# 12334zq/optical-flow-1

Hardware: AMD Instinct MI355X
Metric: Mpix*warp-iters/s, TV-L1 1920x1080 5-scale (higher is better)
Workload: dtype f64; 1 GPU; tvl1flow 1920x1080 pair (synthetic P1), nscales=5 warps=5 tau=0.25 lambda=0.15 theta=0.3 zfactor=0.5 epsilon=0.01; one pair per step per GPU; workload_name=1080p, arithmetic_mode=tolerance, pairs_per_gpu=1040, pairs_in_flight_per_gpu=64, lockstep_group=16, streams_per_gpu=4, distinct_pairs=8

## Files before the change

optical-flow-1_amd/csrc/ofx_ctx.cpp:

```cpp
#include "ofx_internal.h"

#include <cstdarg>
#include <cstdlib>
#include <new>

static const size_t kSlabAlign = 256;
static const size_t kMinSlab = 32u << 20;
static const size_t kMaxSlabs = 24;

int ofx_fail(ofx_ctx *ctx, int status, const char *fmt, ...)
{
    if (ctx) {
        va_list ap;
        va_start(ap, fmt);
        vsnprintf(ctx->errmsg, sizeof(ctx->errmsg), fmt, ap);
        va_end(ap);
    }
    return status;
}

extern "C" const char *ofx_strerror(int status)
{
    switch (status) {
    case OFX_OK:        return "ok";
// ... 47 lines not shown
    ctx->rows_per_wave = 0;
    ctx->rows_per_wave2 = 0;
    ctx->fuse2 = 1;
    ctx->store_a = 1;
    ctx->concurrency = 1;
    ctx->lockstep = 0;
    ctx->warp_lds = 1;
    ctx->gauss_fused = 1;
    ctx->relaxed_dual = 0;
    ctx->tile = 0;
    ctx->tile_max_px = 0;
    ctx->nt_stores = 0;
    ctx->chunk = 0;
    ctx->spin_us = 150;
    ctx->rows_slots = 0;
    ctx->rof_pipe = 1;
    ctx->rof_window = 0;
    ctx->chi_fuse = 1;
    ctx->fuse3 = 2;
    ctx->fuse3_min_px = 0.0;
    ctx->fuse3_cursor = 1;
    ctx->fuse3_afac1 = 0;
    ctx->fuse3_afac2 = 0;
    ctx->rows_per_wave3 = 0;
    ctx->rows3_max = 32;
    ctx->fixed_work = 0;
    ctx->sor_exact = 1;
    ctx->sor_batch = 0;
    ctx->sor_fuse = 0;
    ctx->sor_tile = 0;
    ctx->sor_tile_w = 0;
    ctx->sor_wave_levels = 1;
    ctx->sor_wave_p = 0;
    ctx->sor_window = 0;
    ctx->sor_rows = 0;
    ctx->sor_spw = 0;
    ctx->sor_lds = 1;
    ctx->mem_budget = 0;
    ctx->input = OFX_IN_STORAGE;
    ctx->input_vec = 1;
    ctx->input_lut = 1;
    ctx->poll_seq = 0;
    ctx->errmsg[0] = 0;
    ctx->expo_host_ms = 0.0;
    memset(&ctx->stats, 0, sizeof(ctx->stats));

// ... 167 lines not shown
    if (!strcmp(name, "input_vec")) { ctx->input_vec = value != 0; return OFX_OK; }
    if (!strcmp(name, "input_lut")) { ctx->input_lut = value != 0; return OFX_OK; }
    if (!strcmp(name, "fuse2")) { ctx->fuse2 = value != 0; return OFX_OK; }
    if (!strcmp(name, "store_a")) {
        if (value != 0 && value != 1 && value != 2) return ofx_fail(ctx, OFX_ERR_ARG, "store_a must be 0, 1 or 2");
        ctx->store_a = (int) value;
        return OFX_OK;
    }
    if (!strcmp(name, "rows_slots")) { ctx->rows_slots = (int) value; return OFX_OK; }
    if (!strcmp(name, "rof_pipe")) { ctx->rof_pipe = value != 0; return OFX_OK; }
    if (!strcmp(name, "rof_window")) {
        if (value != 0 && value != 24 && value != 10) return ofx_fail(ctx, OFX_ERR_ARG, "rof_window must be 0, 10 or 24");
        ctx->rof_window = (int) value;
        return OFX_OK;
    }
    if (!strcmp(name, "chi_fuse")) { ctx->chi_fuse = value != 0; return OFX_OK; }
    if (!strcmp(name, "fuse3")) {
        if (value != 0 && value != 1 && value != 2) return ofx_fail(ctx, OFX_ERR_ARG, "fuse3 must be 0, 1 or 2");
        ctx->fuse3 = (int) value;
        return OFX_OK;
    }
    if (!strcmp(name, "fuse3_min_px")) { ctx->fuse3_min_px = value; return OFX_OK; }
    if (!strcmp(name, "fuse3_cursor")) { ctx->fuse3_cursor = value != 0; return OFX_OK; }
    if (!strcmp(name, "fuse3_afac1")) { ctx->fuse3_afac1 = value; return value >= 0 ? OFX_OK : ofx_fail(ctx, OFX_ERR_ARG, "fuse3_afac1 < 0"); }
    if (!strcmp(name, "fuse3_afac2")) { ctx->fuse3_afac2 = value; return value >= 0 ? OFX_OK : ofx_fail(ctx, OFX_ERR_ARG, "fuse3_afac2 < 0"); }
    if (!strcmp(name, "rows_per_wave3")) { ctx->rows_per_wave3 = (int) value; return OFX_OK; }
    if (!strcmp(name, "rows3_max")) { ctx->rows3_max = (int) value; return OFX_OK; }
    if (!strcmp(name, "spin_us")) {
        if (value < 0 || value > 1e6) return ofx_fail(ctx, OFX_ERR_ARG, "spin_us out of range");
        ctx->spin_us = (int) value;
        return OFX_OK;
    }
    if (!strcmp(name, "chunk")) {
        if (value < 0 || value > OFX_TVL1_MAX_ITERATIONS) return ofx_fail(ctx, OFX_ERR_ARG, "chunk out of range");
        ctx->chunk = (int) value;
        return OFX_OK;
    }
    return ofx_fail(ctx, OFX_ERR_ARG, "unknown option '%s'", name);
}

extern "C" int ofx_get_stats(const ofx_ctx *ctx, ofx_stats *out)
{
    if (!ctx || !out) return OFX_ERR_ARG;
    *out = ctx->stats;
    return OFX_OK;
}

void ofx_arena_reset(ofx_ctx *ctx)
// ... 47 lines not shown
```

optical-flow-1_amd/csrc/ofx_internal.h:

```cpp
#pragma once

#include <hip/hip_runtime.h>

#include <cstddef>
#include <cstdint>
#include <cstdio>
#include <cstring>
#include <chrono>
#include <vector>

#include "ofx.h"

#define OFX_NSHARD 64
#define OFX_NPOLL  4
#define OFX_MAX_GROUP 16

struct OfxIterState {
    int    n;
    int    done;
    double error;
    int    apred;
    int    seq;
    int    unit, k0, ucnt;
};
// ... 29 lines not shown
    OfxIterState *h_state;
    double       *h_aux;
    hipEvent_t    ev_poll[OFX_NPOLL];
    hipEvent_t    ev_t0, ev_t1;

    int profile;
    int rows_per_wave;
    int rows_per_wave2;
    int fuse2;
    int store_a;
    int concurrency;
    int lockstep;
    int nt_stores;
    int relaxed_dual;
    int tile;
    double tile_max_px;
    int gauss_fused;
    int warp_lds;
    int chunk;
    int fuse3;
    double fuse3_min_px;
    int fuse3_cursor;
    double fuse3_afac1, fuse3_afac2;
    int rows_per_wave3;
    int rows3_max;
    int chi_fuse;
    int rof_window;
    int rof_pipe;
    int rows_slots;
    int spin_us;
    int fixed_work;
    int sor_exact;
    int sor_fuse;
    int sor_tile;
    int sor_tile_w;
    int sor_wave_p;
    int sor_wave_levels;
    int sor_batch;
    int sor_window;
    int sor_rows;
    int sor_lds;
    int sor_spw;
    int input;
    int input_vec;
    int input_lut;
    double mem_budget;
// ... 73 lines not shown
```

optical-flow-1_amd/csrc/ofx_tvl1.hip:

```cpp
#include "ofx_ops.h"
#include "ofx_device.h"
#include "ofx_loop.h"

#include <atomic>
#include <chrono>
#include <cmath>
#include <thread>

#define TVL1_GRAD_IS_ZERO 1E-10
#define TVL1_PRESMOOTHING_SIGMA 0.8
#define STRIP_OUT 62

template <typename T> OFX_DEV double rnd_to(double x);
template <> OFX_DEV double rnd_to<double>(double x) { return x; }
template <> OFX_DEV double rnd_to<float>(double x) { return (double) (float) x; }

#ifdef OFX_NO_RFL
#define OFX_WAVE_UNIFORM(x) (x)
#else
#define OFX_WAVE_UNIFORM(x) __builtin_amdgcn_readfirstlane(x)
#endif
template <typename T> struct RowIn {
    double2 u, p1, p2, a;
    double r;
// ... 432 lines not shown
    RowIn<T> cur;
    if (!idle) {
        if (ys > 0) {
            up12 = ldw2(at(P1in, off - row2)).y;
            up22 = ldw2(at(P2in, off - row2)).y;
        }
        cur = tvl1_load_row<T>(Uin, P1in, P2in, A, R, off);
    }
    double e1;
    if (!tvl1_continues(prev1, prev2, k, nx * ny, eps2, e1)) return;
    if (idle) return;
    if (((amask >> g) & 1u) || tvl1_store_a(k, e1, eps2, afac))
        tvl1_iter2_march<T, NT, true, STRICT>(Uin, P1in, P2in, A, R, hu.out, h1.out, h2.out, hu.alt, h1.alt, h2.alt, err, k, gw, nx, ny,
                                      y0, yend, ys, yl, lef, rig, owner, off, so, up12, up22, cur, l_t, theta, taut);
    else
        tvl1_iter2_march<T, NT, false, STRICT>(Uin, P1in, P2in, A, R, hu.out, h1.out, h2.out, hu.alt, h1.alt, h2.alt, err, k, gw, nx, ny,
                                       y0, yend, ys, yl, lef, rig, owner, off, so, up12, up22, cur, l_t, theta, taut);
}

#ifndef STRIP3_OUT
#define STRIP3_OUT 56
#endif
#define STRIP3_HALO ((64 - STRIP3_OUT) / 2)
#ifndef OFX_ITER3_WAVES
#define OFX_ITER3_WAVES 3
#endif
template <typename T, bool NT, bool STRICT, int CNT>
OFX_DEV void tvl1_iter3_march(const typename Pix<T>::v2 *__restrict__ Uin, const typename Pix<T>::v2 *__restrict__ P1in,
                              const typename Pix<T>::v2 *__restrict__ P2in, const typename Pix<T>::v2 *__restrict__ A,
                              const T *__restrict__ R, typename Pix<T>::v2 *Uout, typename Pix<T>::v2 *P1out,
                              typename Pix<T>::v2 *P2out, double *__restrict__ err, int slot0, int slot_step, int gw, int nx,
                              int ny, int y0, int yend, int ys, int yl, bool lef, bool rig, bool owner, unsigned off, unsigned so,
                              double up12, double up22, RowIn<T> cur, double l_t, double theta, double taut)
{
    const unsigned E2 = 2 * sizeof(T);
    const unsigned row2 = (unsigned) nx * E2;
    const double2 z2 = make_double2(0.0, 0.0);
    const unsigned level_bytes = (unsigned) nx * (unsigned) ny * E2;
    const ofx_rsrc rU = make_rsrc(Uout, level_bytes), rP1 = make_rsrc(P1out, level_bytes), rP2 = make_rsrc(P2out, level_bytes);
    double accA = 0.0, accB = 0.0, accC = 0.0;
    double2 uA0 = z2, uA1 = z2, uA2 = z2;
    double2 a1 = z2, a2 = z2, a3 = z2, a4 = z2;
    double r1c = 0.0, r2c = 0.0, r3c = 0.0, r4c = 0.0;
    double2 p0a = z2, p0b = z2;
    double2 pA1a = z2, pA1b = z2, pA2a = z2, pA2b = z2;
    double2 uB0 = z2, uB1 = z2, uB2 = z2;
    double2 pB1a = z2, pB1b = z2, pB2a = z2, pB2b = z2;
    double2 uC0 = z2, uC1 = z2;
    const int nyl = ny - 1;
    const int yB0 = y0 > 0 ? y0 - 1 : 0;
    const int ylc = (yend + CNT - 1 < yl) ? yend + CNT - 1 : yl;
    const int hiA = (yend + CNT - 2 < nyl) ? yend + CNT - 2 : nyl;
    const int hiB = (yend + CNT - 3 < nyl) ? yend + CNT - 3 : nyl;
    const int hiC = (yend < nyl) ? yend : nyl;
    const int ylast = yend - 1 + (2 * CNT - 1);
#ifdef OFX_CEIL_ALU
    const unsigned off0 = off;
#endif

    auto step = [&](const int y) {
        RowIn<T> nxt = cur;
#ifdef OFX_CEIL_ALU
        if (y + 1 <= ylc) nxt = tvl1_load_row<T>(Uin, P1in, P2in, A, R, off0 + ((y & 1) ? row2 : 0u));
#else
        if (y + 1 <= ylc) nxt = tvl1_load_row<T>(Uin, P1in, P2in, A, R, off + row2);
#endif
        unsigned stu = OFX_OOB, stp = OFX_OOB;
        double2 su = z2, sp1 = z2, sp2 = z2;

        if (y <= ylc) {
            const double l11 = wave_shift_up(cur.p1.x);
            const double l21 = wave_shift_up(cur.p2.x);
            uA0 = tvl1_primal<T, STRICT>(cur.u, cur.a, cur.r, cur.p1, cur.p2, l11, l21, up12, up22, lef, rig, y == 0, y == nyl, l_t,
                                         theta);
            const bool mine = owner && y >= y0 && y < yend;
            const double dA = (uA0.x - cur.u.x) * (uA0.x - cur.u.x) + (uA0.y - cur.u.y) * (uA0.y - cur.u.y);
            accA += mine ? dA : 0.0;
            if (CNT == 1 && mine) { stu = so; su = uA0; }
        }
        double2 pAna = z2, pAnb = z2;
        if (y - 1 >= ys && y - 1 <= hiA) {
            const double n1 = wave_shift_down(uA1.x);
            const double n2 = wave_shift_down(uA1.y);
            tvl1_dual<T, STRICT>(p0a, p0b, uA1, n1, n2, uA0, rig, y - 1 == nyl, taut, pAna, pAnb);
            pAna.x = rnd_to<T>(pAna.x); pAna.y = rnd_to<T>(pAna.y);
            pAnb.x = rnd_to<T>(pAnb.x); pAnb.y = rnd_to<T>(pAnb.y);
            if (CNT == 1 && owner && y - 1 >= y0 && y - 1 < yend) { stp = so - row2; sp1 = pAna; sp2 = pAnb; }
        }
        double2 pBna = z2, pBnb = z2;
        if (CNT >= 2) {
            if (y - 2 >= yB0 && y - 2 <= hiA) {
                const double l11 = wave_shift_up(pA1a.x);
                const double l21 = wave_shift_up(pA1b.x);
                uB0 = tvl1_primal<T, STRICT>(uA2, a2, r2c, pA1a, pA1b, l11, l21, pA2a.y, pA2b.y, lef, rig, y - 2 == 0, y - 2 == nyl,
                                             l_t, theta);
                const bool mine = owner && y - 2 >= y0 && y - 2 < yend;
                const double dB = (uB0.x - uA2.x) * (uB0.x - uA2.x) + (uB0.y - uA2.y) * (uB0.y - uA2.y);
                accB += mine ? dB : 0.0;
                if (CNT == 2 && mine) { stu = so - 2 * row2; su = uB0; }
            }
            if (y - 3 >= yB0 && y - 3 <= hiB) {
                const double n1 = wave_shift_down(uB1.x);
                const double n2 = wave_shift_down(uB1.y);
                tvl1_dual<T, STRICT>(pA2a, pA2b, uB1, n1, n2, uB0, rig, y - 3 == nyl, taut, pBna, pBnb);
                pBna.x = rnd_to<T>(pBna.x); pBna.y = rnd_to<T>(pBna.y);
                pBnb.x = rnd_to<T>(pBnb.x); pBnb.y = rnd_to<T>(pBnb.y);
                if (CNT == 2 && owner && y - 3 >= y0 && y - 3 < yend) { stp = so - 3 * row2; sp1 = pBna; sp2 = pBnb; }
            }
        }
        if (CNT == 3) {
            if (y - 4 >= y0 && y - 4 <= hiC) {
                const double l11 = wave_shift_up(pB1a.x);
                const double l21 = wave_shift_up(pB1b.x);
                uC0 = tvl1_primal<T, STRICT>(uB2, a4, r4c, pB1a, pB1b, l11, l21, pB2a.y, pB2b.y, lef, rig, y - 4 == 0, y - 4 == nyl,
                                             l_t, theta);
                const bool mine = owner && y - 4 < yend;
                const double dC = (uC0.x - uB2.x) * (uC0.x - uB2.x) + (uC0.y - uB2.y) * (uC0.y - uB2.y);
                accC += mine ? dC : 0.0;
                stu = mine ? so - 4 * row2 : stu;
                su = uC0;
            }
            if (y - 5 >= y0 && y - 5 < yend) {
                const double n1 = wave_shift_down(uC1.x);
                const double n2 = wave_shift_down(uC1.y);
                tvl1_dual<T, STRICT>(pB2a, pB2b, uC1, n1, n2, uC0, rig, y - 5 == nyl, taut, sp1, sp2);
                if (owner) stp = so - 5 * row2;
            }
        }
#ifdef OFX_CEIL_ALU
        stu = OFX_OOB; stp = OFX_OOB;
#endif
        bst2<NT>(rU, stu, su, Uout);
        bst2<NT>(rP1, stp, sp1, P1out);
        bst2<NT>(rP2, stp, sp2, P2out);
        uA2 = uA1; uA1 = uA0;
        a4 = a3; a3 = a2; a2 = a1; a1 = cur.a;
        r4c = r3c; r3c = r2c; r2c = r1c; r1c = cur.r;
        p0a = cur.p1; p0b = cur.p2;
        up12 = cur.p1.y; up22 = cur.p2.y;
        pA2a = pA1a; pA2b = pA1b; pA1a = pAna; pA1b = pAnb;
        uB2 = uB1; uB1 = uB0;
        pB2a = pB1a; pB2b = pB1b; pB1a = pBna; pB1b = pBnb;
        uC1 = uC0;
        cur = nxt;
        off += row2;
        so += row2;
    };
    for (int y = ys; y <= ylast; y++) step(y);
    loop_accumulate(err, slot0, accA, gw);
    if (CNT >= 2) loop_accumulate(err, slot0 + slot_step, accB, gw);
    if (CNT == 3) loop_accumulate(err, slot0 + 2 * slot_step, accC, gw);
}

template <typename T, bool NT, bool STRICT>
__global__ __launch_bounds__(256) __attribute__((amdgpu_waves_per_eu(OFX_ITER3_WAVES, OFX_ITER3_WAVES))) void k_tvl1_iter3(
    Tri<typename Pix<T>::v2> Ut, Tri<typename Pix<T>::v2> P1t, Tri<typename Pix<T>::v2> P2t,
    const typename Pix<T>::v2 *__restrict__ Ag, const T *__restrict__ Rg, double *__restrict__ errg, int k0, int check, int slot0,
    int nx, int ny, int rows, int strips_x, int strips_pad, double l_t, double theta, double taut, double eps2, unsigned incode,
    unsigned runmask, unsigned long long nit, int err_stride, OfxLoopDev *dev, int launch, double afac1, double afac2, int max_iter)
{
    using v2 = typename Pix<T>::v2;
    const int lane = threadIdx.x & 63;
    const int gw = OFX_WAVE_UNIFORM((int) (blockIdx.x * 4 + (threadIdx.x >> 6)));
    const int g = blockIdx.y;
    if (!((runmask >> g) & 1u)) return;
    int niter = (int) ((nit >> (4 * g)) & 15ull);
    const bool scribe = dev && blockIdx.x == 0 && threadIdx.x == 0;
    if (dev) {
        k0 = dev->cursor[launch & 1][g];
        slot0 = k0;
        check = 1;
        if (scribe) {
            dev->ulog[g][launch] = k0;
            dev->cursor[(launch + 1) & 1][g] = k0;
        }
        if (k0 >= max_iter) return;
    }
    const size_t npix = (size_t) nx * ny;
    const TriSel<v2> hu = pick3(Ut, incode, g, npix), h1 = pick3(P1t, incode, g, npix), h2 = pick3(P2t, incode, g, npix);
    const v2 *__restrict__ Uin = hu.in, *__restrict__ P1in = h1.in, *__restrict__ P2in = h2.in;
    const v2 *__restrict__ A = Ag + (size_t) g * npix;
    const T *__restrict__ R = Rg + (size_t) g * npix;
    double *__restrict__ err = errg + (size_t) g * err_stride;
    double prev[3];
#pragma unroll
    for (int i = 0; i < 3; i++) prev[i] = (check && k0 - i > 0) ? loop_fetch_prev(err, k0 - i) : 0.0;

    const int band = gw / strips_pad, strip = gw % strips_pad;
    const int y0 = band * rows;
    const bool idle = (strip >= strips_x) || (y0 >= ny);
    const int yend = (y0 + rows < ny) ? y0 + rows : ny;
    const int ys = y0 > 2 ? y0 - 2 : 0;
    const int yl = (yend + 2 < ny - 1) ? yend + 2 : ny - 1;
    const int c = strip * STRIP3_OUT - STRIP3_HALO + lane;
    const int cc = c < 0 ? 0 : (c > nx - 1 ? nx - 1 : c);
    const bool lef = (c == 0), rig = (c == nx - 1);
    const bool owner = (lane >= STRIP3_HALO) && (lane < STRIP3_OUT + STRIP3_HALO) && (c < nx);
    const unsigned E2 = 2 * sizeof(T);
    const unsigned row2 = (unsigned) nx * E2;
    const unsigned off = ((unsigned) ys * nx + cc) * E2;
    const unsigned so = ((unsigned) ys * nx + (c < 0 ? 0 : c)) * E2;
    double up12 = 0.0, up22 = 0.0;
    RowIn<T> cur;
    if (!idle) {
        if (ys > 0) {
            up12 = ldw2(at(P1in, off - row2)).y;
            up22 = ldw2(at(P2in, off - row2)).y;
        }
        cur = tvl1_load_row<T>(Uin, P1in, P2in, A, R, off);
    }
    if (check) {
        double e1 = 0.0;
#pragma unroll
        for (int i = 0; i < 3; i++) {
            if (k0 - i > 0) {
                const double e = loop_error_from_sum(wave_allreduce_sum(prev[i]), nx * ny, OFX_CRIT_MEAN);
                if (!(e > eps2)) return;
                if (i == 0) e1 = e;
            }
        }
        if (dev) {
            niter = (k0 > 0 && e1 <= eps2 * afac1) ? 1 : ((k0 > 0 && e1 <= eps2 * afac2) ? 2 : 3);
            if (niter > max_iter - k0) niter = max_iter - k0;
            if (scribe) dev->cursor[(launch + 1) & 1][g] = k0 + niter;
        }
    }
    if (idle) return;
    const int step = check ? 1 : 0;
    if (niter >= 3)
        tvl1_iter3_march<T, NT, STRICT, 3>(Uin, P1in, P2in, A, R, hu.out, h1.out, h2.out, err, slot0, step, gw, nx, ny, y0, yend, ys, yl,
                                           lef, rig, owner, off, so, up12, up22, cur, l_t, theta, taut);
    else if (niter == 2)
        tvl1_iter3_march<T, NT, STRICT, 2>(Uin, P1in, P2in, A, R, hu.out, h1.out, h2.out, err, slot0, step, gw, nx, ny, y0, yend, ys, yl,
                                           lef, rig, owner, off, so, up12, up22, cur, l_t, theta, taut);
    else
        tvl1_iter3_march<T, NT, STRICT, 1>(Uin, P1in, P2in, A, R, hu.out, h1.out, h2.out, err, slot0, step, gw, nx, ny, y0, yend, ys, yl,
                                           lef, rig, owner, off, so, up12, up22, cur, l_t, theta, taut);
}

#define TILE_RH 16
template <typename T, bool STRICT, int K>
__global__ __launch_bounds__(64 * TILE_RH) void k_tvl1_tile(
    Tri<typename Pix<T>::v2> Ut, Tri<typename Pix<T>::v2> P1t, Tri<typename Pix<T>::v2> P2t,
    const typename Pix<T>::v2 *__restrict__ Ag, const T *__restrict__ Rg, double *__restrict__ errg, int k0, int check, int slot0,
    int nx, int ny, int tiles_x, double l_t, double theta, double taut, double eps2, unsigned incode, unsigned runmask,
    unsigned long long nit, int err_stride)
{
    using v2 = typename Pix<T>::v2;
    static_assert(K < 16, "4 bits of `nit` per pair");
    __shared__ double2 s_p[2][TILE_RH][64];
    __shared__ double2 s_u[2][TILE_RH][64];
    const int lane = threadIdx.x & 63, w = threadIdx.x >> 6;
    const int g = blockIdx.y;
    if (!((runmask >> g) & 1u)) return;
    const int niter = (int) ((nit >> (4 * g)) & 15ull);
    const size_t npix = (size_t) nx * ny;
    const TriSel<v2> hu = pick3(Ut, incode, g, npix), h1 = pick3(P1t, incode, g, npix), h2 = pick3(P2t, incode, g, npix);
    double *__restrict__ err = errg + (size_t) g * err_stride;
    double prev[K];
#pragma unroll
// ... 305 lines not shown

static int tvl1_pick_chunk(const ofx_ctx *ctx, int nx, int ny, int G)
{
    if (ctx->chunk > 0) return ctx->chunk;
    const double est_us = fmax(5.0, (double) nx * ny * G * 120.0 / 4.0e6);
    int c = (int) (40.0 / est_us);
    return c < 4 ? 4 : (c > 50 ? 50 : c);
}

static int tvl1_pick_tile(const ofx_ctx *ctx, int nx, int ny, int G)
{
    if (!ctx->tile || !ctx->fuse2) return 0;
    const double lim = ctx->tile_max_px > 0 ? ctx->tile_max_px : 200000.0;
    if ((double) nx * ny * G > lim) return 0;
    return ctx->tile == 6 ? 6 : 4;
}

template <typename T> struct Tvl1Level;
struct Tvl1Params;
template <typename T>
static int tvl1_run_iterations_tile(ofx_ctx *ctx, Tvl1Level<T> &L, const Tvl1Params &P, LoopSpec S, int K, int *n_out,
                                    double *err_out, float *ms_out, int *alt_out);
template <typename T>
static int tvl1_run_iterations_tri(ofx_ctx *ctx, Tvl1Level<T> &L, const Tvl1Params &P, LoopSpec S, int *n_out, double *err_out,
                                   float *ms_out, int *alt_out);

static int tvl1_pick_rows3(const ofx_ctx *ctx, int nx, int ny, int G)
{
    if (ctx->rows_per_wave3 > 0) return ctx->rows_per_wave3;
    {
        static const char *tab = getenv("OFX_ROWS3");
        for (const char *q = tab; q && *q;) {
            int lny = 0, r = 0;
            if (sscanf(q, "%d:%d", &lny, &r) == 2 && lny == ny && r > 0) return r;
            q = strchr(q, '/');
            if (q) q++;
        }
    }
    const long strips_pad = (long) ofx_cdiv(ofx_cdiv(nx, STRIP3_OUT), 4) * 4 * G;
    const int rmax = 32;
    int best = rmax;
    long best_cost = -1;
    if (ctx->concurrency > 1) {
        static const int cand[] = {2, 3, 4, 5, 6, 8, 10, 12, 14, 16, 20, 24, 28, 32, 36, 40, 48, 54, 64, 72, 80, 96};
        for (int r : cand) {
            if (r > ctx->rows3_max) break;
            const long waves = strips_pad * ofx_cdiv(ny, r);
            const long slots = ctx->rows_slots > 0 ? ctx->rows_slots : 1024;
            const long cost = ((waves + slots - 1) / slots) * (r + 7);
            if (best_cost < 0 || cost < best_cost) { best_cost = cost; best = r; }
        }
        return best;
    }
    const long slots = 1024L * OFX_ITER3_WAVES;
    for (int k = 1; k <= 4; k++) {
        for (int r = 1; r <= rmax; r++) {
            if (strips_pad * ofx_cdiv(ny, r) > k * slots) continue;
            const long cost = (long) k * (r + 7);
            if (best_cost < 0 || cost < best_cost) { best_cost = cost; best = r; }
            break;
        }
    }
    if (best < 4 && strips_pad * ofx_cdiv(ny, 4) >= 512) best = 4;
    return best;
}

template <typename T>
static int tvl1_run_iterations(ofx_ctx *ctx, Tvl1Level<T> &L, const Tvl1Params &P, int *n_out, double *err_out,
                               float *ms_out, int *alt_out = nullptr,
                               int *unit_out = nullptr)
{
    const int nx = L.nx, ny = L.ny, G = L.G;
    if ((long long) nx * ny >= (1LL << 27)) return ofx_fail(ctx, OFX_ERR_ARG, "tvl1: image larger than 2^27 pixels");
    const double l_t = P.lambda * P.theta, taut = P.tau / P.theta, theta = P.theta;
    const bool pairs = ctx->fuse2 != 0;
    const int rows = tvl1_pick_rows(ctx, nx, ny, G);
    const int strips_x = ofx_cdiv(nx, STRIP_OUT), strips_pad = ofx_cdiv(strips_x, 4) * 4;
    const unsigned gx1 = (unsigned) (strips_pad / 4) * ofx_cdiv(ny, rows);
    const dim3 block(256);
    const int rows2 = tvl1_pick_rows2(ctx, nx, ny, G);
    const int strips2_x = ofx_cdiv(nx, STRIP2_OUT), strips2_pad = ofx_cdiv(strips2_x, 4) * 4;
    const dim3 grid2((unsigned) (strips2_pad / 4) * ofx_cdiv(ny, rows2), G);
    LoopSpec S;
    S.max_iter = P.max_iter;
    S.size = nx * ny;
    S.thr = P.epsilon * P.epsilon;
    S.crit = OFX_CRIT_MEAN;
    S.chunk = tvl1_pick_chunk(ctx, nx, ny, G);
    S.fixed = P.fixed;
    S.pairs = pairs;
    const int tileK = tvl1_pick_tile(ctx, nx, ny, G);
    if (unit_out) *unit_out = tileK ? tileK : (pairs ? 2 : 1);
    if (tileK) return tvl1_run_iterations_tile<T>(ctx, L, P, S, tileK, n_out, err_out, ms_out, alt_out);
    {
        const bool strict_mode = sizeof(T) == sizeof(double) && !ctx->relaxed_dual;
        const double px = (double) nx * ny * G;
        const bool tri = ctx->fuse3 == 1 ? px >= ctx->fuse3_min_px
                                         : (ctx->fuse3 == 2 && !strict_mode && (G >= 2 || ctx->concurrency > 1) &&
                                            px >= (ctx->fuse3_min_px > 0 ? ctx->fuse3_min_px : 5e5));
        if (pairs && tri) {
            if (unit_out) *unit_out = 3;
            return tvl1_run_iterations_tri<T>(ctx, L, P, S, n_out, err_out, ms_out, alt_out);
        }
    }
    const int err_stride = (S.max_iter + 1) * OFX_NSHARD;
    const unsigned all = (G >= 32) ? 0xFFFFFFFFu : ((1u << G) - 1u);
    const bool nt_stores = ctx->nt_stores ? ctx->nt_stores == 1 : (double) nx * ny * G * 15.0 * sizeof(T) > 300e6;
    unsigned b0[OFX_MAX_GROUP];
    for (int g = 0; g < G; g++) b0[g] = L.curidx(g);
    auto code_of = [&](unsigned unit) -> unsigned {
        unsigned c = 0;
        for (int g = 0; g < G; g++) c |= ((b0[g] + unit) % 3u) << (2 * g);
        return c;
    };
    const bool sa = pairs && !P.fixed && ctx->store_a != 0;
    S.afac = sa ? (ctx->store_a == 2 ? 1e300 : 1.5) : 0.0;
    unsigned amask0 = 0;
    if (sa)
        for (int g = 0; g < G; g++)
            if (ctx->store_a == 2 || (L.last_n[g] >= 1 && L.last_n[g] <= 2)) amask0 |= 1u << g;
    const bool strict = sizeof(T) == sizeof(double) && !ctx->relaxed_dual;
    auto single = [&](unsigned incode, unsigned runmask, int check, int slot, double thr) -> int {
        auto kern = k_tvl1_iter<T, false>;
        if constexpr (sizeof(T) == sizeof(double)) { if (strict) kern = k_tvl1_iter<T, true>; }
        hipLaunchKernelGGL(kern, dim3(gx1, G), block, 0, ctx->stream, L.Ut(), L.P1t(), L.P2t(), L.A, (const T *) L.R,
// ... 82 lines not shown
        for (int g = 0; g < G; g++) {
            if (k_of[g] < 0) continue;
            const int n = k_of[g] + 1, j = (n - 1) / K;
            runmask |= 1u << g;
            incode |= ((b0[g] + (unsigned) j) % 3u) << (2 * g);
            nit |= (unsigned long long) (n - j * K) << (4 * g);
        }
        return go(0, 0, S.max_iter, -1.0, incode, runmask, nit);
    };
    int took_alt[OFX_MAX_GROUP];
    OFX_TRY(ofx_run_loop_group(ctx, S, G, launch, redo, n_out, err_out, ms_out, 0u, took_alt));
    unsigned cur = 0;
    for (int g = 0; g < G; g++) {
        const unsigned units = (unsigned) ((n_out[g] + K - 1) / K);
        cur |= ((b0[g] + units) % 3u) << (2 * g);
        L.last_n[g] = n_out[g];
        if (alt_out) alt_out[g] = 0;
    }
    L.cur = cur;
    return OFX_OK;
}

template <typename T>
static int tvl1_run_iterations_tri(ofx_ctx *ctx, Tvl1Level<T> &L, const Tvl1Params &P, LoopSpec S, int *n_out, double *err_out,
                                   float *ms_out, int *alt_out)
{
    const int nx = L.nx, ny = L.ny, G = L.G;
    const double l_t = P.lambda * P.theta, taut = P.tau / P.theta, theta = P.theta;
    const bool strict = sizeof(T) == sizeof(double) && !ctx->relaxed_dual;
    const int rows = tvl1_pick_rows3(ctx, nx, ny, G);
    const int strips_x = ofx_cdiv(nx, STRIP3_OUT), strips_pad = ofx_cdiv(strips_x, 4) * 4;
    const dim3 grid((unsigned) (strips_pad / 4) * ofx_cdiv(ny, rows), G), block(256);
    const bool nt_stores = ctx->nt_stores ? ctx->nt_stores == 1 : (double) nx * ny * G * 15.0 * sizeof(T) > 300e6;
    S.pairs = false;
    S.fuse = 3;
    S.afac = 0.0;
    const int err_stride = (S.max_iter + 1) * OFX_NSHARD;
    const unsigned all = (G >= 32) ? 0xFFFFFFFFu : ((1u << G) - 1u);
    unsigned b0[OFX_MAX_GROUP];
    for (int g = 0; g < G; g++) b0[g] = L.curidx(g);
    const bool cursor = ctx->fuse3_cursor != 0 && !S.fixed;
    const double afac2 = ctx->fuse3_afac2 > 0 ? ctx->fuse3_afac2 : 1.5, afac1 = ctx->fuse3_afac1 > 0 ? ctx->fuse3_afac1 : 1.2;
    auto go = [&](int k0, int check, int slot0, double thr, unsigned incode, unsigned runmask, unsigned long long nit, OfxLoopDev *dev,
                  int launch) -> int {
        auto kern = nt_stores ? k_tvl1_iter3<T, true, false> : k_tvl1_iter3<T, false, false>;
        if constexpr (sizeof(T) == sizeof(double)) {
            if (strict) kern = nt_stores ? k_tvl1_iter3<T, true, true> : k_tvl1_iter3<T, false, true>;
        }
        hipLaunchKernelGGL(kern, grid, block, 0, ctx->stream, L.Ut(), L.P1t(), L.P2t(), L.A, (const T *) L.R, ctx->d_err, k0, check,
                           slot0, nx, ny, rows, strips_x, strips_pad, l_t, theta, taut, thr, incode, runmask, nit, err_stride, dev, launch,
                           afac1, afac2, S.max_iter);
        OFX_LAUNCH_CHECK(ctx);
        return OFX_OK;
    };
    auto code_of_unit = [&](unsigned unit) -> unsigned {
        unsigned c = 0;
        for (int g = 0; g < G; g++) c |= ((b0[g] + unit) % 3u) << (2 * g);
        return c;
    };
    int unit_of[OFX_MAX_GROUP];
    int inside[OFX_MAX_GROUP];
    if (cursor) {
        auto launch = [&](int Lidx, double thr) -> int {
            return go(0, 1, 0, thr, code_of_unit((unsigned) Lidx), all, 0ull, reinterpret_cast<OfxLoopDev *>(ctx->d_state), Lidx);
        };
        auto redo = [&](const int *n_of, const int *k0_of, const int *u_of) -> int {
            unsigned incode = 0, runmask = 0;
            unsigned long long nit = 0;
            for (int g = 0; g < G; g++) {
                if (n_of[g] < 0) continue;
                runmask |= 1u << g;
                incode |= ((b0[g] + (unsigned) u_of[g]) % 3u) << (2 * g);
                nit |= (unsigned long long) (n_of[g] - k0_of[g]) << (4 * g);
            }
            return go(0, 0, S.max_iter, -1.0, incode, runmask, nit, nullptr, 0);
        };
        const int upc = (S.chunk + 2) / 3 < 1 ? 1 : (S.chunk + 2) / 3;
        OFX_TRY(ofx_run_loop_cursor(ctx, S, G, upc, 3, launch, redo, n_out, err_out, unit_of, inside, ms_out));
    } else {
        auto launch = [&](int k, int cnt, double thr) -> int {
            unsigned long long nit = 0;
            for (int g = 0; g < G; g++) nit |= (unsigned long long) cnt << (4 * g);
            return go(k, 1, k, thr, code_of_unit((unsigned) (k / 3)), all, nit, nullptr, 0);
        };
        auto redo = [&](const int *k_of) -> int {
            unsigned incode = 0, runmask = 0;
            unsigned long long nit = 0;
            for (int g = 0; g < G; g++) {
                if (k_of[g] < 0) continue;
                const int n = k_of[g] + 1, j = (n - 1) / 3;
                runmask |= 1u << g;
                incode |= ((b0[g] + (unsigned) j) % 3u) << (2 * g);
                nit |= (unsigned long long) (n - j * 3) << (4 * g);
            }
            return go(0, 0, S.max_iter, -1.0, incode, runmask, nit, nullptr, 0);
        };
        int took_alt[OFX_MAX_GROUP];
        OFX_TRY(ofx_run_loop_group(ctx, S, G, launch, redo, n_out, err_out, ms_out, 0u, took_alt));
        for (int g = 0; g < G; g++) {
            unit_of[g] = n_out[g] > 0 ? (n_out[g] - 1) / 3 : -1;
            inside[g] = (n_out[g] % 3 != 0 && n_out[g] != S.max_iter) ? 1 : 0;
        }
    }
    unsigned cur = 0;
    for (int g = 0; g < G; g++) {
        const unsigned units = (unsigned) (unit_of[g] + 1);
        cur |= ((b0[g] + units) % 3u) << (2 * g);
        L.last_n[g] = n_out[g];
        if (alt_out) alt_out[g] = inside[g] ? 1 : 0;
    }
    L.cur = cur;
    return OFX_OK;
}

template <typename T>
static int tvl1_single_scale_dev(ofx_ctx *ctx, Tvl1Level<T> &L, const Tvl1Params &P, int scale, ofx_stats *stats)
{
    const int nx = L.nx, ny = L.ny, G = L.G;
    const size_t n = L.n();
    const dim3 g2(ofx_cdiv(nx, OFX_WARP_BX), ofx_cdiv(ny, OFX_WARP_BY), G), b2(OFX_WARP_BX, OFX_WARP_BY);
    if (nx < 2 || ny < 2) return ofx_fail(ctx, OFX_ERR_ARG, "tvl1: level %dx%d too small", nx, ny);

    OFX_TRY(op_grad_pack<T>(ctx, L.I1, L.pa, L.pb, nx, ny, G));
    for (int h = 0; h < 3; h++) {
// ... 476 lines not shown
```

Measured before the change: 76480 Mpix*warp-iters/s.

## Add four-iteration fused TV-L1 march kernel with LDS ring for data terms

Extends the temporally fused row-marching TV-L1 iteration from three to four primal/dual iterations per launch. A new k_tvl1_iter4 kernel keeps the A and R data terms of recent rows in a shared-memory ring instead of a register shift chain, which lets it add a fourth pipeline stage with its own halo rows and error accumulator. It is selected by default for levels of at least about two million pixels when the three-iteration path would be used. The intent is to cut global memory round trips and launches per iteration, at the cost of deeper row halos (more redundant computation), extra register pressure and LDS traffic, and a coarser convergence-check granularity.

Result: faster. 78440 Mpix*warp-iters/s, median of 6 (+2.6%).

```diff
diff --git a/optical-flow-1_amd/csrc/ofx_ctx.cpp b/optical-flow-1_amd/csrc/ofx_ctx.cpp
--- a/optical-flow-1_amd/csrc/ofx_ctx.cpp
+++ b/optical-flow-1_amd/csrc/ofx_ctx.cpp
@@ -93,6 +93,9 @@
     ctx->fuse3_cursor = 1;
     ctx->fuse3_afac1 = 0;
     ctx->fuse3_afac2 = 0;
+    ctx->fuse4 = 2;
+    ctx->fuse4_min_px = 0.0;
+    ctx->fuse4_afac3 = 0;
     ctx->rows_per_wave3 = 0;
     ctx->rows3_max = 32;
     ctx->fixed_work = 0;
@@ -306,8 +309,21 @@
     }
     if (!strcmp(name, "fuse3_min_px")) { ctx->fuse3_min_px = value; return OFX_OK; }
     if (!strcmp(name, "fuse3_cursor")) { ctx->fuse3_cursor = value != 0; return OFX_OK; }
-    if (!strcmp(name, "fuse3_afac1")) { ctx->fuse3_afac1 = value; return value >= 0 ? OFX_OK : ofx_fail(ctx, OFX_ERR_ARG, "fuse3_afac1 < 0"); }
-    if (!strcmp(name, "fuse3_afac2")) { ctx->fuse3_afac2 = value; return value >= 0 ? OFX_OK : ofx_fail(ctx, OFX_ERR_ARG, "fuse3_afac2 < 0"); }
+    if (!strcmp(name, "fuse3_afac1") || !strcmp(name, "fuse3_afac2") || !strcmp(name, "fuse4_afac3")) {
+        if (!(value >= 0)) return ofx_fail(ctx, OFX_ERR_ARG, "%s < 0", name);
+        (name[10] == '1' ? ctx->fuse3_afac1 : (name[10] == '2' ? ctx->fuse3_afac2 : ctx->fuse4_afac3)) = value;
+        return OFX_OK;
+    }
+    if (!strcmp(name, "fuse4")) {
+        if (value != 0 && value != 1 && value != 2) return ofx_fail(ctx, OFX_ERR_ARG, "fuse4 must be 0, 1 or 2");
+        ctx->fuse4 = (int) value;
+        return OFX_OK;
+    }
+    if (!strcmp(name, "fuse4_min_px")) {
+        if (!(value >= 0)) return ofx_fail(ctx, OFX_ERR_ARG, "fuse4_min_px < 0");
+        ctx->fuse4_min_px = value;
+        return OFX_OK;
+    }
     if (!strcmp(name, "rows_per_wave3")) { ctx->rows_per_wave3 = (int) value; return OFX_OK; }
     if (!strcmp(name, "rows3_max")) { ctx->rows3_max = (int) value; return OFX_OK; }
     if (!strcmp(name, "spin_us")) {
diff --git a/optical-flow-1_amd/csrc/ofx_internal.h b/optical-flow-1_amd/csrc/ofx_internal.h
--- a/optical-flow-1_amd/csrc/ofx_internal.h
+++ b/optical-flow-1_amd/csrc/ofx_internal.h
@@ -75,6 +75,9 @@
     double fuse3_min_px;
     int fuse3_cursor;
     double fuse3_afac1, fuse3_afac2;
+    int fuse4;
+    double fuse4_min_px;
+    double fuse4_afac3;
     int rows_per_wave3;
     int rows3_max;
     int chi_fuse;
diff --git a/optical-flow-1_amd/csrc/ofx_tvl1.hip b/optical-flow-1_amd/csrc/ofx_tvl1.hip
--- a/optical-flow-1_amd/csrc/ofx_tvl1.hip
+++ b/optical-flow-1_amd/csrc/ofx_tvl1.hip
@@ -478,23 +478,31 @@
 #define STRIP3_OUT 56
 #endif
 #define STRIP3_HALO ((64 - STRIP3_OUT) / 2)
+#define TVL1_RING_ROWS 8
+struct Tvl1Ring {
+    double2 a[TVL1_RING_ROWS][64];
+    double  r[TVL1_RING_ROWS][64];
+};
 #ifndef OFX_ITER3_WAVES
 #define OFX_ITER3_WAVES 3
 #endif
-template <typename T, bool NT, bool STRICT, int CNT>
+template <typename T, bool NT, bool STRICT, int CNT, int N>
 OFX_DEV void tvl1_iter3_march(const typename Pix<T>::v2 *__restrict__ Uin, const typename Pix<T>::v2 *__restrict__ P1in,
                               const typename Pix<T>::v2 *__restrict__ P2in, const typename Pix<T>::v2 *__restrict__ A,
                               const T *__restrict__ R, typename Pix<T>::v2 *Uout, typename Pix<T>::v2 *P1out,
                               typename Pix<T>::v2 *P2out, double *__restrict__ err, int slot0, int slot_step, int gw, int nx,
                               int ny, int y0, int yend, int ys, int yl, bool lef, bool rig, bool owner, unsigned off, unsigned so,
-                              double up12, double up22, RowIn<T> cur, double l_t, double theta, double taut)
-{
+                              double up12, double up22, RowIn<T> cur, double l_t, double theta, double taut,
+                              Tvl1Ring *ring = nullptr)
+{
+    static_assert(CNT >= 1 && CNT <= N && (N == 3 || N == 4), "units of up to three or four iterations");
+    constexpr bool RING = CNT == 4;
     const unsigned E2 = 2 * sizeof(T);
     const unsigned row2 = (unsigned) nx * E2;
     const double2 z2 = make_double2(0.0, 0.0);
     const unsigned level_bytes = (unsigned) nx * (unsigned) ny * E2;
     const ofx_rsrc rU = make_rsrc(Uout, level_bytes), rP1 = make_rsrc(P1out, level_bytes), rP2 = make_rsrc(P2out, level_bytes);
-    double accA = 0.0, accB = 0.0, accC = 0.0;
+    double accA = 0.0, accB = 0.0, accC = 0.0, accD = 0.0;
     double2 uA0 = z2, uA1 = z2, uA2 = z2;
     double2 a1 = z2, a2 = z2, a3 = z2, a4 = z2;
     double r1c = 0.0, r2c = 0.0, r3c = 0.0, r4c = 0.0;
@@ -502,14 +510,18 @@
     double2 pA1a = z2, pA1b = z2, pA2a = z2, pA2b = z2;
     double2 uB0 = z2, uB1 = z2, uB2 = z2;
     double2 pB1a = z2, pB1b = z2, pB2a = z2, pB2b = z2;
-    double2 uC0 = z2, uC1 = z2;
+    double2 uC0 = z2, uC1 = z2, uC2 = z2;
+    double2 pC1a = z2, pC1b = z2, pC2a = z2, pC2b = z2;
+    double2 uD0 = z2, uD1 = z2;
     const int nyl = ny - 1;
-    const int yB0 = y0 > 0 ? y0 - 1 : 0;
+    const int yB0 = y0 > N - 2 ? y0 - (N - 2) : 0;
+    const int yC0 = y0 > N - 3 ? y0 - (N - 3) : 0;
     const int ylc = (yend + CNT - 1 < yl) ? yend + CNT - 1 : yl;
     const int hiA = (yend + CNT - 2 < nyl) ? yend + CNT - 2 : nyl;
     const int hiB = (yend + CNT - 3 < nyl) ? yend + CNT - 3 : nyl;
-    const int hiC = (yend < nyl) ? yend : nyl;
+    const int hiC = (yend + CNT - 4 < nyl) ? yend + CNT - 4 : nyl;
     const int ylast = yend - 1 + (2 * CNT - 1);
+    unsigned ri = 0;
 #ifdef OFX_CEIL_ALU
     const unsigned off0 = off;
 #endif
@@ -543,12 +555,20 @@
             pAnb.x = rnd_to<T>(pAnb.x); pAnb.y = rnd_to<T>(pAnb.y);
             if (CNT == 1 && owner && y - 1 >= y0 && y - 1 < yend) { stp = so - row2; sp1 = pAna; sp2 = pAnb; }
         }
+        [[maybe_unused]] const int lane = threadIdx.x & 63;
+        if constexpr (RING) {
+            ring->a[ri][lane] = cur.a;
+            ring->r[ri][lane] = cur.r;
+        }
         double2 pBna = z2, pBnb = z2;
         if (CNT >= 2) {
             if (y - 2 >= yB0 && y - 2 <= hiA) {
+                double2 ad = a2;
+                double rd = r2c;
+                if constexpr (RING) { ad = ring->a[(ri - 2u) % TVL1_RING_ROWS][lane]; rd = ring->r[(ri - 2u) % TVL1_RING_ROWS][lane]; }
                 const double l11 = wave_shift_up(pA1a.x);
                 const double l21 = wave_shift_up(pA1b.x);
-                uB0 = tvl1_primal<T, STRICT>(uA2, a2, r2c, pA1a, pA1b, l11, l21, pA2a.y, pA2b.y, lef, rig, y - 2 == 0, y - 2 == nyl,
+                uB0 = tvl1_primal<T, STRICT>(uA2, ad, rd, pA1a, pA1b, l11, l21, pA2a.y, pA2b.y, lef, rig, y - 2 == 0, y - 2 == nyl,
                                              l_t, theta);
                 const bool mine = owner && y - 2 >= y0 && y - 2 < yend;
                 const double dB = (uB0.x - uA2.x) * (uB0.x - uA2.x) + (uB0.y - uA2.y) * (uB0.y - uA2.y);
@@ -564,23 +584,56 @@
                 if (CNT == 2 && owner && y - 3 >= y0 && y - 3 < yend) { stp = so - 3 * row2; sp1 = pBna; sp2 = pBnb; }
             }
         }
-        if (CNT == 3) {
-            if (y - 4 >= y0 && y - 4 <= hiC) {
+        double2 pCna = z2, pCnb = z2;
+        if (CNT >= 3) {
+            if (y - 4 >= yC0 && y - 4 <= hiB) {
+                double2 ad = a4;
+                double rd = r4c;
+                if constexpr (RING) { ad = ring->a[(ri - 4u) % TVL1_RING_ROWS][lane]; rd = ring->r[(ri - 4u) % TVL1_RING_ROWS][lane]; }
                 const double l11 = wave_shift_up(pB1a.x);
                 const double l21 = wave_shift_up(pB1b.x);
-                uC0 = tvl1_primal<T, STRICT>(uB2, a4, r4c, pB1a, pB1b, l11, l21, pB2a.y, pB2b.y, lef, rig, y - 4 == 0, y - 4 == nyl,
+                uC0 = tvl1_primal<T, STRICT>(uB2, ad, rd, pB1a, pB1b, l11, l21, pB2a.y, pB2b.y, lef, rig, y - 4 == 0, y - 4 == nyl,
                                              l_t, theta);
-                const bool mine = owner && y - 4 < yend;
+                const bool mine = owner && y - 4 >= y0 && y - 4 < yend;
                 const double dC = (uC0.x - uB2.x) * (uC0.x - uB2.x) + (uC0.y - uB2.y) * (uC0.y - uB2.y);
                 accC += mine ? dC : 0.0;
-                stu = mine ? so - 4 * row2 : stu;
-                su = uC0;
+                if (CNT == 3) {
+                    stu = mine ? so - 4 * row2 : stu;
+                    su = uC0;
+                }
             }
-            if (y - 5 >= y0 && y - 5 < yend) {
+            if (y - 5 >= yC0 && y - 5 <= hiC) {
                 const double n1 = wave_shift_down(uC1.x);
                 const double n2 = wave_shift_down(uC1.y);
-                tvl1_dual<T, STRICT>(pB2a, pB2b, uC1, n1, n2, uC0, rig, y - 5 == nyl, taut, sp1, sp2);
-                if (owner) stp = so - 5 * row2;
+                tvl1_dual<T, STRICT>(pB2a, pB2b, uC1, n1, n2, uC0, rig, y - 5 == nyl, taut, pCna, pCnb);
+                if (CNT == 3) {
+                    sp1 = pCna; sp2 = pCnb;
+                    if (owner && y - 5 >= y0) stp = so - 5 * row2;
+                } else {
+                    pCna.x = rnd_to<T>(pCna.x); pCna.y = rnd_to<T>(pCna.y);
+                    pCnb.x = rnd_to<T>(pCnb.x); pCnb.y = rnd_to<T>(pCnb.y);
+                }
+            }
+        }
+        if constexpr (CNT == 4) {
+            if (y - 6 >= y0 && y - 6 <= hiC) {
+                const double2 ad = ring->a[(ri - 6u) % TVL1_RING_ROWS][lane];
+                const double rd = ring->r[(ri - 6u) % TVL1_RING_ROWS][lane];
+                const double l11 = wave_shift_up(pC1a.x);
+                const double l21 = wave_shift_up(pC1b.x);
+                uD0 = tvl1_primal<T, STRICT>(uC2, ad, rd, pC1a, pC1b, l11, l21, pC2a.y, pC2b.y, lef, rig, y - 6 == 0, y - 6 == nyl,
+                                             l_t, theta);
+                const bool mine = owner && y - 6 < yend;
+                const double dD = (uD0.x - uC2.x) * (uD0.x - uC2.x) + (uD0.y - uC2.y) * (uD0.y - uC2.y);
+                accD += mine ? dD : 0.0;
+                stu = mine ? so - 6 * row2 : stu;
+                su = uD0;
+            }
+            if (y - 7 >= y0 && y - 7 < yend) {
+                const double n1 = wave_shift_down(uD1.x);
+                const double n2 = wave_shift_down(uD1.y);
+                tvl1_dual<T, STRICT>(pC2a, pC2b, uD1, n1, n2, uD0, rig, y - 7 == nyl, taut, sp1, sp2);
+                if (owner) stp = so - 7 * row2;
             }
         }
 #ifdef OFX_CEIL_ALU
@@ -590,14 +643,20 @@
         bst2<NT>(rP1, stp, sp1, P1out);
         bst2<NT>(rP2, stp, sp2, P2out);
         uA2 = uA1; uA1 = uA0;
-        a4 = a3; a3 = a2; a2 = a1; a1 = cur.a;
-        r4c = r3c; r3c = r2c; r2c = r1c; r1c = cur.r;
+        if constexpr (RING) {
+            ri = (ri + 1u) % TVL1_RING_ROWS;
+        } else {
+            a4 = a3; a3 = a2; a2 = a1; a1 = cur.a;
+            r4c = r3c; r3c = r2c; r2c = r1c; r1c = cur.r;
+        }
         p0a = cur.p1; p0b = cur.p2;
         up12 = cur.p1.y; up22 = cur.p2.y;
         pA2a = pA1a; pA2b = pA1b; pA1a = pAna; pA1b = pAnb;
         uB2 = uB1; uB1 = uB0;
         pB2a = pB1a; pB2b = pB1b; pB1a = pBna; pB1b = pBnb;
-        uC1 = uC0;
+        uC2 = uC1; uC1 = uC0;
+        pC2a = pC1a; pC2b = pC1b; pC1a = pCna; pC1b = pCnb;
+        uD1 = uD0;
         cur = nxt;
         off += row2;
         so += row2;
@@ -605,15 +664,16 @@
     for (int y = ys; y <= ylast; y++) step(y);
     loop_accumulate(err, slot0, accA, gw);
     if (CNT >= 2) loop_accumulate(err, slot0 + slot_step, accB, gw);
-    if (CNT == 3) loop_accumulate(err, slot0 + 2 * slot_step, accC, gw);
-}
-
-template <typename T, bool NT, bool STRICT>
-__global__ __launch_bounds__(256) __attribute__((amdgpu_waves_per_eu(OFX_ITER3_WAVES, OFX_ITER3_WAVES))) void k_tvl1_iter3(
-    Tri<typename Pix<T>::v2> Ut, Tri<typename Pix<T>::v2> P1t, Tri<typename Pix<T>::v2> P2t,
-    const typename Pix<T>::v2 *__restrict__ Ag, const T *__restrict__ Rg, double *__restrict__ errg, int k0, int check, int slot0,
-    int nx, int ny, int rows, int strips_x, int strips_pad, double l_t, double theta, double taut, double eps2, unsigned incode,
-    unsigned runmask, unsigned long long nit, int err_stride, OfxLoopDev *dev, int launch, double afac1, double afac2, int max_iter)
+    if (CNT >= 3) loop_accumulate(err, slot0 + 2 * slot_step, accC, gw);
+    if (CNT == 4) loop_accumulate(err, slot0 + 3 * slot_step, accD, gw);
+}
+
+template <typename T, bool NT, bool STRICT, int N>
+OFX_DEV void tvl1_unit(Tri<typename Pix<T>::v2> Ut, Tri<typename Pix<T>::v2> P1t, Tri<typename Pix<T>::v2> P2t,
+                       const typename Pix<T>::v2 *__restrict__ Ag, const T *__restrict__ Rg, double *__restrict__ errg, int k0,
+                       int check, int slot0, int nx, int ny, int rows, int strips_x, int strips_pad, double l_t, double theta,
+                       double taut, double eps2, unsigned incode, unsigned runmask, unsigned long long nit, int err_stride,
+                       OfxLoopDev *dev, int launch, double afac1, double afac2, double afac3, int max_iter, Tvl1Ring *ring)
 {
     using v2 = typename Pix<T>::v2;
     const int lane = threadIdx.x & 63;
@@ -638,16 +698,16 @@
     const v2 *__restrict__ A = Ag + (size_t) g * npix;
     const T *__restrict__ R = Rg + (size_t) g * npix;
     double *__restrict__ err = errg + (size_t) g * err_stride;
-    double prev[3];
+    double prev[N];
 #pragma unroll
-    for (int i = 0; i < 3; i++) prev[i] = (check && k0 - i > 0) ? loop_fetch_prev(err, k0 - i) : 0.0;
+    for (int i = 0; i < N; i++) prev[i] = (check && k0 - i > 0) ? loop_fetch_prev(err, k0 - i) : 0.0;
 
     const int band = gw / strips_pad, strip = gw % strips_pad;
     const int y0 = band * rows;
     const bool idle = (strip >= strips_x) || (y0 >= ny);
     const int yend = (y0 + rows < ny) ? y0 + rows : ny;
-    const int ys = y0 > 2 ? y0 - 2 : 0;
-    const int yl = (yend + 2 < ny - 1) ? yend + 2 : ny - 1;
+    const int ys = y0 > N - 1 ? y0 - (N - 1) : 0;
+    const int yl = (yend + N - 1 < ny - 1) ? yend + N - 1 : ny - 1;
     const int c = strip * STRIP3_OUT - STRIP3_HALO + lane;
     const int cc = c < 0 ? 0 : (c > nx - 1 ? nx - 1 : c);
     const bool lef = (c == 0), rig = (c == nx - 1);
@@ -668,7 +728,7 @@
     if (check) {
         double e1 = 0.0;
 #pragma unroll
-        for (int i = 0; i < 3; i++) {
+        for (int i = 0; i < N; i++) {
             if (k0 - i > 0) {
                 const double e = loop_error_from_sum(wave_allreduce_sum(prev[i]), nx * ny, OFX_CRIT_MEAN);
                 if (!(e > eps2)) return;
@@ -677,21 +737,51 @@
         }
         if (dev) {
             niter = (k0 > 0 && e1 <= eps2 * afac1) ? 1 : ((k0 > 0 && e1 <= eps2 * afac2) ? 2 : 3);
+            if (N == 4 && niter == 3 && !(k0 > 0 && e1 <= eps2 * afac3)) niter = 4;
             if (niter > max_iter - k0) niter = max_iter - k0;
             if (scribe) dev->cursor[(launch + 1) & 1][g] = k0 + niter;
         }
     }
     if (idle) return;
     const int step = check ? 1 : 0;
-    if (niter >= 3)
-        tvl1_iter3_march<T, NT, STRICT, 3>(Uin, P1in, P2in, A, R, hu.out, h1.out, h2.out, err, slot0, step, gw, nx, ny, y0, yend, ys, yl,
-                                           lef, rig, owner, off, so, up12, up22, cur, l_t, theta, taut);
+    if (N == 4 && niter >= 4) {
+        if constexpr (N == 4)
+            tvl1_iter3_march<T, NT, STRICT, 4, N>(Uin, P1in, P2in, A, R, hu.out, h1.out, h2.out, err, slot0, step, gw, nx, ny, y0, yend,
+                                                  ys, yl, lef, rig, owner, off, so, up12, up22, cur, l_t, theta, taut, ring);
+    } else if (niter >= 3)
+        tvl1_iter3_march<T, NT, STRICT, 3, N>(Uin, P1in, P2in, A, R, hu.out, h1.out, h2.out, err, slot0, step, gw, nx, ny, y0, yend, ys,
+                                              yl, lef, rig, owner, off, so, up12, up22, cur, l_t, theta, taut);
     else if (niter == 2)
-        tvl1_iter3_march<T, NT, STRICT, 2>(Uin, P1in, P2in, A, R, hu.out, h1.out, h2.out, err, slot0, step, gw, nx, ny, y0, yend, ys, yl,
-                                           lef, rig, owner, off, so, up12, up22, cur, l_t, theta, taut);
+        tvl1_iter3_march<T, NT, STRICT, 2, N>(Uin, P1in, P2in, A, R, hu.out, h1.out, h2.out, err, slot0, step, gw, nx, ny, y0, yend, ys,
+                                              yl, lef, rig, owner, off, so, up12, up22, cur, l_t, theta, taut);
     else
-        tvl1_iter3_march<T, NT, STRICT, 1>(Uin, P1in, P2in, A, R, hu.out, h1.out, h2.out, err, slot0, step, gw, nx, ny, y0, yend, ys, yl,
-                                           lef, rig, owner, off, so, up12, up22, cur, l_t, theta, taut);
+        tvl1_iter3_march<T, NT, STRICT, 1, N>(Uin, P1in, P2in, A, R, hu.out, h1.out, h2.out, err, slot0, step, gw, nx, ny, y0, yend, ys,
+                                              yl, lef, rig, owner, off, so, up12, up22, cur, l_t, theta, taut);
+}
+
+template <typename T, bool NT, bool STRICT>
+__global__ __launch_bounds__(256) __attribute__((amdgpu_waves_per_eu(OFX_ITER3_WAVES, OFX_ITER3_WAVES))) void k_tvl1_iter3(
+    Tri<typename Pix<T>::v2> Ut, Tri<typename Pix<T>::v2> P1t, Tri<typename Pix<T>::v2> P2t,
+    const typename Pix<T>::v2 *__restrict__ Ag, const T *__restrict__ Rg, double *__restrict__ errg, int k0, int check, int slot0,
+    int nx, int ny, int rows, int strips_x, int strips_pad, double l_t, double theta, double taut, double eps2, unsigned incode,
+    unsigned runmask, unsigned long long nit, int err_stride, OfxLoopDev *dev, int launch, double afac1, double afac2, double afac3,
+    int max_iter)
+{
+    tvl1_unit<T, NT, STRICT, 3>(Ut, P1t, P2t, Ag, Rg, errg, k0, check, slot0, nx, ny, rows, strips_x, strips_pad, l_t, theta, taut, eps2,
+                                incode, runmask, nit, err_stride, dev, launch, afac1, afac2, afac3, max_iter, nullptr);
+}
+
+template <typename T, bool NT, bool STRICT>
+__global__ __launch_bounds__(256) __attribute__((amdgpu_waves_per_eu(OFX_ITER3_WAVES, OFX_ITER3_WAVES))) void k_tvl1_iter4(
+    Tri<typename Pix<T>::v2> Ut, Tri<typename Pix<T>::v2> P1t, Tri<typename Pix<T>::v2> P2t,
+    const typename Pix<T>::v2 *__restrict__ Ag, const T *__restrict__ Rg, double *__restrict__ errg, int k0, int check, int slot0,
+    int nx, int ny, int rows, int strips_x, int strips_pad, double l_t, double theta, double taut, double eps2, unsigned incode,
+    unsigned runmask, unsigned long long nit, int err_stride, OfxLoopDev *dev, int launch, double afac1, double afac2, double afac3,
+    int max_iter)
+{
+    __shared__ Tvl1Ring rings[4];
+    tvl1_unit<T, NT, STRICT, 4>(Ut, P1t, P2t, Ag, Rg, errg, k0, check, slot0, nx, ny, rows, strips_x, strips_pad, l_t, theta, taut, eps2,
+                                incode, runmask, nit, err_stride, dev, launch, afac1, afac2, afac3, max_iter, &rings[threadIdx.x >> 6]);
 }
 
 #define TILE_RH 16
@@ -1043,11 +1133,12 @@
 static int tvl1_run_iterations_tile(ofx_ctx *ctx, Tvl1Level<T> &L, const Tvl1Params &P, LoopSpec S, int K, int *n_out,
                                     double *err_out, float *ms_out, int *alt_out);
 template <typename T>
-static int tvl1_run_iterations_tri(ofx_ctx *ctx, Tvl1Level<T> &L, const Tvl1Params &P, LoopSpec S, int *n_out, double *err_out,
+static int tvl1_run_iterations_tri(ofx_ctx *ctx, Tvl1Level<T> &L, const Tvl1Params &P, LoopSpec S, int N, int *n_out, double *err_out,
                                    float *ms_out, int *alt_out);
 
-static int tvl1_pick_rows3(const ofx_ctx *ctx, int nx, int ny, int G)
-{
+static int tvl1_pick_rows3(const ofx_ctx *ctx, int nx, int ny, int G, int N = 3)
+{
+    const int depth = 2 * N + 1;
     if (ctx->rows_per_wave3 > 0) return ctx->rows_per_wave3;
     {
         static const char *tab = getenv("OFX_ROWS3");
@@ -1068,7 +1159,7 @@
             if (r > ctx->rows3_max) break;
             const long waves = strips_pad * ofx_cdiv(ny, r);
             const long slots = ctx->rows_slots > 0 ? ctx->rows_slots : 1024;
-            const long cost = ((waves + slots - 1) / slots) * (r + 7);
+            const long cost = ((waves + slots - 1) / slots) * (r + depth);
             if (best_cost < 0 || cost < best_cost) { best_cost = cost; best = r; }
         }
         return best;
@@ -1077,7 +1168,7 @@
     for (int k = 1; k <= 4; k++) {
         for (int r = 1; r <= rmax; r++) {
             if (strips_pad * ofx_cdiv(ny, r) > k * slots) continue;
-            const long cost = (long) k * (r + 7);
+            const long cost = (long) k * (r + depth);
             if (best_cost < 0 || cost < best_cost) { best_cost = cost; best = r; }
             break;
         }
@@ -1086,6 +1177,9 @@
     return best;
 }
 
+#ifndef TVL1_FUSE4_AUTO_PX
+#define TVL1_FUSE4_AUTO_PX 2e6
+#endif
 template <typename T>
 static int tvl1_run_iterations(ofx_ctx *ctx, Tvl1Level<T> &L, const Tvl1Params &P, int *n_out, double *err_out,
                                float *ms_out, int *alt_out = nullptr,
@@ -1119,9 +1213,12 @@
         const bool tri = ctx->fuse3 == 1 ? px >= ctx->fuse3_min_px
                                          : (ctx->fuse3 == 2 && !strict_mode && (G >= 2 || ctx->concurrency > 1) &&
                                             px >= (ctx->fuse3_min_px > 0 ? ctx->fuse3_min_px : 5e5));
-        if (pairs && tri) {
-            if (unit_out) *unit_out = 3;
-            return tvl1_run_iterations_tri<T>(ctx, L, P, S, n_out, err_out, ms_out, alt_out);
+        const bool quad = ctx->fuse4 == 1 ? px >= ctx->fuse4_min_px
+                                          : (ctx->fuse4 == 2 && tri && ctx->fuse3 == 2 &&
+                                             px >= (ctx->fuse4_min_px > 0 ? ctx->fuse4_min_px : TVL1_FUSE4_AUTO_PX));
+        if (pairs && (tri || quad)) {
+            if (unit_out) *unit_out = quad ? 4 : 3;
+            return tvl1_run_iterations_tri<T>(ctx, L, P, S, quad ? 4 : 3, n_out, err_out, ms_out, alt_out);
         }
     }
     const int err_stride = (S.max_iter + 1) * OFX_NSHARD;
@@ -1250,18 +1347,18 @@
 }
 
 template <typename T>
-static int tvl1_run_iterations_tri(ofx_ctx *ctx, Tvl1Level<T> &L, const Tvl1Params &P, LoopSpec S, int *n_out, double *err_out,
+static int tvl1_run_iterations_tri(ofx_ctx *ctx, Tvl1Level<T> &L, const Tvl1Params &P, LoopSpec S, int N, int *n_out, double *err_out,
                                    float *ms_out, int *alt_out)
 {
     const int nx = L.nx, ny = L.ny, G = L.G;
     const double l_t = P.lambda * P.theta, taut = P.tau / P.theta, theta = P.theta;
     const bool strict = sizeof(T) == sizeof(double) && !ctx->relaxed_dual;
-    const int rows = tvl1_pick_rows3(ctx, nx, ny, G);
+    const int rows = tvl1_pick_rows3(ctx, nx, ny, G, N);
     const int strips_x = ofx_cdiv(nx, STRIP3_OUT), strips_pad = ofx_cdiv(strips_x, 4) * 4;
     const dim3 grid((unsigned) (strips_pad / 4) * ofx_cdiv(ny, rows), G), block(256);
     const bool nt_stores = ctx->nt_stores ? ctx->nt_stores == 1 : (double) nx * ny * G * 15.0 * sizeof(T) > 300e6;
     S.pairs = false;
-    S.fuse = 3;
+    S.fuse = N;
     S.afac = 0.0;
     const int err_stride = (S.max_iter + 1) * OFX_NSHARD;
     const unsigned all = (G >= 32) ? 0xFFFFFFFFu : ((1u << G) - 1u);
@@ -1269,15 +1366,18 @@
     for (int g = 0; g < G; g++) b0[g] = L.curidx(g);
     const bool cursor = ctx->fuse3_cursor != 0 && !S.fixed;
     const double afac2 = ctx->fuse3_afac2 > 0 ? ctx->fuse3_afac2 : 1.5, afac1 = ctx->fuse3_afac1 > 0 ? ctx->fuse3_afac1 : 1.2;
+    const double afac3 = ctx->fuse4_afac3 > 0 ? ctx->fuse4_afac3 : afac2;
     auto go = [&](int k0, int check, int slot0, double thr, unsigned incode, unsigned runmask, unsigned long long nit, OfxLoopDev *dev,
                   int launch) -> int {
         auto kern = nt_stores ? k_tvl1_iter3<T, true, false> : k_tvl1_iter3<T, false, false>;
+        if (N == 4) kern = nt_stores ? k_tvl1_iter4<T, true, false> : k_tvl1_iter4<T, false, false>;
         if constexpr (sizeof(T) == sizeof(double)) {
             if (strict) kern = nt_stores ? k_tvl1_iter3<T, true, true> : k_tvl1_iter3<T, false, true>;
+            if (strict && N == 4) kern = nt_stores ? k_tvl1_iter4<T, true, true> : k_tvl1_iter4<T, false, true>;
         }
         hipLaunchKernelGGL(kern, grid, block, 0, ctx->stream, L.Ut(), L.P1t(), L.P2t(), L.A, (const T *) L.R, ctx->d_err, k0, check,
                            slot0, nx, ny, rows, strips_x, strips_pad, l_t, theta, taut, thr, incode, runmask, nit, err_stride, dev, launch,
-                           afac1, afac2, S.max_iter);
+                           afac1, afac2, afac3, S.max_iter);
         OFX_LAUNCH_CHECK(ctx);
         return OFX_OK;
     };
@@ -1303,31 +1403,31 @@
             }
             return go(0, 0, S.max_iter, -1.0, incode, runmask, nit, nullptr, 0);
         };
-        const int upc = (S.chunk + 2) / 3 < 1 ? 1 : (S.chunk + 2) / 3;
-        OFX_TRY(ofx_run_loop_cursor(ctx, S, G, upc, 3, launch, redo, n_out, err_out, unit_of, inside, ms_out));
+        const int upc = (S.chunk + N - 1) / N < 1 ? 1 : (S.chunk + N - 1) / N;
+        OFX_TRY(ofx_run_loop_cursor(ctx, S, G, upc, N, launch, redo, n_out, err_out, unit_of, inside, ms_out));
     } else {
         auto launch = [&](int k, int cnt, double thr) -> int {
             unsigned long long nit = 0;
             for (int g = 0; g < G; g++) nit |= (unsigned long long) cnt << (4 * g);
-            return go(k, 1, k, thr, code_of_unit((unsigned) (k / 3)), all, nit, nullptr, 0);
+            return go(k, 1, k, thr, code_of_unit((unsigned) (k / N)), all, nit, nullptr, 0);
         };
         auto redo = [&](const int *k_of) -> int {
             unsigned incode = 0, runmask = 0;
             unsigned long long nit = 0;
             for (int g = 0; g < G; g++) {
                 if (k_of[g] < 0) continue;
-                const int n = k_of[g] + 1, j = (n - 1) / 3;
+                const int n = k_of[g] + 1, j = (n - 1) / N;
                 runmask |= 1u << g;
                 incode |= ((b0[g] + (unsigned) j) % 3u) << (2 * g);
-                nit |= (unsigned long long) (n - j * 3) << (4 * g);
+                nit |= (unsigned long long) (n - j * N) << (4 * g);
             }
             return go(0, 0, S.max_iter, -1.0, incode, runmask, nit, nullptr, 0);
         };
         int took_alt[OFX_MAX_GROUP];
         OFX_TRY(ofx_run_loop_group(ctx, S, G, launch, redo, n_out, err_out, ms_out, 0u, took_alt));
         for (int g = 0; g < G; g++) {
-            unit_of[g] = n_out[g] > 0 ? (n_out[g] - 1) / 3 : -1;
-            inside[g] = (n_out[g] % 3 != 0 && n_out[g] != S.max_iter) ? 1 : 0;
+            unit_of[g] = n_out[g] > 0 ? (n_out[g] - 1) / N : -1;
+            inside[g] = (n_out[g] % N != 0 && n_out[g] != S.max_iter) ? 1 : 0;
         }
     }
     unsigned cur = 0;
```
